# stevenabreu7/SparseRNNs

Hardware: AMD Instinct MI355X
Metric: frames/sec at w8a16 S5 dim_scale=0.5 (NDNS shape), bit-exact vs CPU fxprun (higher is better)
Workload: dtype int32

## Files before the change

sparsernns_amd/csrc/mfma_fused_body.inc:

```
    CGateArgs a = a_k;
    {
        const int64_t g = blockIdx.y;
        gshift(a.u, g * go.ws); gshift(a.skip, g * go.ws); gshift(a.xs, g * go.ws); gshift(a.z, g * go.ws);
        gshift(a.skip_e.dyn, g * go.ws); gshift(a.dynw, g * go.ws); gshift(a.run_if, g * go.ws); gshift(a.status, g * go.status);
        if constexpr (GBN || UREC) { gshift(a.bn.dyn, g * go.ws); gshift(a.bn.xe.dyn, g * go.ws); }
    }
    static_assert(!GBN || (PK16 && !TRACE && !WIDE), "the BatchNorm rides on the packed-epilogue kernel only");
    static_assert(!UREC || (PK16 && !TRACE && !WIDE && !GBN), "u is rebuilt in the row tiles' staging: COAL only");
    constexpr int P = 32 * KS, H = shape_channels(NT), HP = 32 * NT, FT = FTP, NW = (FT / 32) * NT, NTHR = 64 * NW;
    constexpr bool RAGGED = H != HP;
    constexpr int KPS = 2 * P + 16, KPX = HP + 16;
    constexpr int NU = 1, SUBSTEP = 0;
    constexpr int ITEMS = (FT / 4) * P, ROUNDS = (ITEMS + NTHR - 1) / NTHR;
    extern __shared__ __attribute__((aligned(16))) int8_t smem[];
    int32_t *csr = reinterpret_cast<int32_t *>(smem), *csi = csr + HP, *Dl = csi + HP, *cs2 = Dl + HP, *be = cs2 + HP, *lutp = be + HP;
    int32_t *sigt = lutp + 8;
    const int16_t *sigd = reinterpret_cast<const int16_t *>(sigt);
    constexpr int NPL = WIDE ? 4 : 2;
    int8_t *Sbase = reinterpret_cast<int8_t *>(sigt) + (DIRECT ? sigdir_lds_bytes(a.sigdir_bits) : 4 * SIGTAB_WORDS);
    int8_t *Sl = Sbase, *Sh = Sbase + (NPL - 1) * FT * KPS, *Xh = Sbase + NPL * FT * KPS, *Xl = Xh + FT * KPX;
    float *red = reinterpret_cast<float *>(Xl + FT * KPX);
    int32_t *bntab = reinterpret_cast<int32_t *>(red + 48);
    constexpr bool COAL = PK16 && !TRACE && !WIDE && !GBN;
    constexpr int TROW = 2 * HP + 8, VPF = H / 8, NVC = (FT * VPF + NTHR - 1) / NTHR;
    constexpr bool NVC_FULL = FT * VPF % NTHR == 0;
    static_assert(!COAL || NVC_FULL || RAGGED, "tile vectors per thread");
    static_assert(!UREC || NTHR % VPF == 0, "a thread's channel group must be the same for every vector");
    static_assert(!FOLD || (UREC && !RAGGED), "the aligned sum is formed in the UREC staging");
    int8_t *Ut = reinterpret_cast<int8_t *>(red + 48), *St = Ut + FT * TROW;
    const int l = threadIdx.x & 63, r = l & 31, h = l >> 5, wave = threadIdx.x >> 6;
    const int ct = wave % NT, sub0 = wave / NT;
    const StepRange sr{a.t_lo, a.t_len};
    const int64_t tiles = (a.N / a.L) * ((sr.t_len + FT - 1) / FT);
    if (WIDE && a.run_if && *a.run_if == 0) return;

    v4i wre[KS], wim[KS], wo2[NT];
    {
        const size_t row = (size_t)(32 * ct + r);
#pragma unroll
        for (int ks = 0; ks < KS; ++ks) {
            wre[ks] = *reinterpret_cast<const v4i *>(a.w_re.wt + row * a.w_re.Kp + 32 * ks + 16 * h);
            wim[ks] = *reinterpret_cast<const v4i *>(a.w_im.wt + row * a.w_im.Kp + 32 * ks + 16 * h);
        }
#pragma unroll
        for (int ks = 0; ks < NT; ++ks) wo2[ks] = *reinterpret_cast<const v4i *>(a.w_o2.wt + row * a.w_o2.Kp + 32 * ks + 16 * h);
    }
    for (int i = threadIdx.x; i < HP; i += NTHR) {
        csr[i] = a.w_re.cs128[i]; csi[i] = a.w_im.cs128[i]; Dl[i] = a.D[i]; cs2[i] = a.w_o2.cs128[i];
        if (!PK16) be[i] = a.bias_eff[i];
    }
    if (PK16)
        for (int i = threadIdx.x; i < HP / 2; i += NTHR)
            be[i] = (int32_t)(((uint32_t)a.bias_eff[2 * i] & 0xffffu) | ((uint32_t)a.bias_eff[2 * i + 1] << 16));
    if (threadIdx.x < 8) lutp[threadIdx.x] = a_k.lut[threadIdx.x] | (a_k.lut[threadIdx.x < 7 ? threadIdx.x + 1 : 7] << 16);
    if (DIRECT) {
        for (int i = threadIdx.x; i < (1 << a.sigdir_bits) / 2; i += NTHR)
            sigt[i] = reinterpret_cast<const int32_t *>(a.sigdir)[i];
    } else {
        for (int i = threadIdx.x; i < (14 << a.sig_x); i += NTHR) sigt[i] = a.sigtab[i];
    }
    Bn16 bn{};
    if constexpr (GBN) bn = bn16_setup(a.bn, *a.bn.dyn, bntab, H);
    std::conditional_t<UREC, Bn16Row, int> brow{};
    if constexpr (UREC) brow = bn16_row_setup(a.bn, *a.bn.dyn, 8 * (int)(threadIdx.x % VPF));
    [[maybe_unused]] v4i *brow_lds = reinterpret_cast<v4i *>(St + FT * TROW);
    if constexpr (FOLD) {
        if (threadIdx.x < VPF) {
            brow_lds[2 * threadIdx.x] = v4i{(int)brow.m[0], (int)brow.m[1], (int)brow.m[2], (int)brow.m[3]};
            brow_lds[2 * threadIdx.x + 1] = v4i{(int)brow.iv[0], (int)brow.iv[1], (int)brow.iv[2], (int)brow.iv[3]};
        }
    }
    const int dsh = a.out_exp - a.sig_x, dbias = 1 << (a.sigdir_bits - 1);
    const int skip_e = a.skip_e.get();
    const float kz = ldexpf(1.f, skip_e - a.res_exp);
    const v4i *usum_lds = reinterpret_cast<const v4i *>(red + 8);
    if constexpr (FOLD) {
        if (threadIdx.x == 0) {
            const SumU16 us = sum_u16_setup_exps(a.res_exp, skip_e);
            *reinterpret_cast<v4i *>(red + 8) = v4i{(int)us.mz, (int)us.mz2, (int)us.ms, (int)us.ms2};
            const LayerDyn *sd = skip_dyn_of(a_k);
            gshift(sd, (int64_t)blockIdx.y * go.ws);
            const ResolveU16 rz = resolve_u16_setup(sd ? sd->res.post : 0);
            *reinterpret_cast<v4i *>(red + 12) = v4i{(int)rz.shr, (int)rz.m1, (int)rz.m2, sd ? 1 : 0};
        }
    }
    auto resolve_skip = [&](v4i &sv) {
        const v4i rw = *reinterpret_cast<const v4i *>(red + 12);
        if (__builtin_amdgcn_readfirstlane(rw[3])) {
            const ResolveU16 rz{(uint32_t)rw[0], (uint32_t)rw[1], (uint32_t)rw[2], RES_GENERIC};
#pragma unroll
            for (int q = 0; q < 4; ++q) sv[q] = (int)resolve_u16_pair<RES_GENERIC>(rz, (uint32_t)sv[q]);
        }
    };
    const int sx = a.sig_x, S = 1 << sx;
    const int cv_l = a.conv && a.inp_exp > a.y_exp ? a.inp_exp - a.y_exp : 0, cv_r = a.conv && a.y_exp > a.inp_exp ? a.y_exp - a.inp_exp : 0;
    const int cv_b1 = a.conv && a.inp_exp != a.y_exp ? a.y_bits : 32, cv_b2 = a.conv && a.y_bits > a.inp_bits ? a.inp_bits : 32;
    const int cv_b = cv_b1 < cv_b2 ? cv_b1 : cv_b2;
    const int lq_l = a.l_exp > a.y_exp ? a.l_exp - a.y_exp : 0, lq_r = a.y_exp > a.l_exp ? a.y_exp - a.l_exp : 0;
    uint32_t xrange = 0;
    v2i16 pmax = {0, 0}, pmin = {0, 0};
    float mx[3] = {0.f, 0.f, 0.f};
    const int ch0 = 32 * ct + 4 * h;
    v2i uq[NU][4], sq[NU][4];
    v4i urow[COAL && !UREC ? NVC : 1], srow[COAL ? NVC : 1];
    auto load_tile = [&](v4i(&dst)[COAL ? NVC : 1], const int16_t *src, const TileWalk<FT> &tw) {
        const int64_t b = tw.b;
        const int t = tw.t(sr), nv = tw.nvalid(sr);
        const char *base = reinterpret_cast<const char *>(src + (b * a.L + t) * H);
#pragma unroll
        for (int i = 0; i < NVC; ++i) {
            const int v = threadIdx.x + NTHR * i;
            if (!NVC_FULL && v >= FT * VPF) break;
            int f = v / VPF;
            f = f < nv ? f : nv - 1;
            dst[i] = *reinterpret_cast<const v4i *>(base + 2u * (unsigned)(f * H + 8 * (v % VPF)));
        }
    };
    auto load_rows = [&](v2i(&dst)[NU][4], const int16_t *src, const TileWalk<FT> &tw) {
        const int64_t b = tw.b;
        const int t = tw.t(sr), nv = tw.nvalid(sr);
        const char *base = reinterpret_cast<const char *>(src + (b * a.L + t) * H);
#pragma unroll
        for (int u = 0; u < NU; ++u) {
            int fo = 32 * (sub0 + u * SUBSTEP) + r;
            fo = fo < nv ? fo : nv - 1;
            const unsigned fb = 2u * (unsigned)(fo * H + ch0);
#pragma unroll
            for (int g = 0; g < 4; ++g) {
                if (RAGGED && ch0 + 8 * g >= H) dst[u][g] = v2i{0, 0};
                else dst[u][g] = *reinterpret_cast<const v2i *>(base + fb + 16 * g);
            }
        }
    };
    if constexpr (COAL && RAGGED) {
        for (int i = threadIdx.x; i < 2 * FT; i += NTHR) {
            int8_t *t = Ut + i * TROW + 2 * H;
#pragma unroll
            for (int j = 0; j < (HP - H) / 4; ++j) *reinterpret_cast<v2i *>(t + 8 * j) = v2i{0, 0};
        }
    }
    TileWalk<FT> walk((int64_t)blockIdx.x, sr, gridDim.x);
    if ((int64_t)blockIdx.x < tiles) {
        if constexpr (COAL) {
            if constexpr (!UREC) load_tile(urow, a.u, walk);
            load_tile(srow, a.skip, walk);
        } else {
            if constexpr (!GBN) load_rows(uq, a.u, walk);
            load_rows(sq, a.skip, walk);
        }
    }
    __syncthreads();
    char *zb_prev = nullptr;
    int nvalid_prev = 0;
    auto fold_z = [&](v2i &z0, v2i &z1, const int8_t *cs_) {
        const v2i s0 = *reinterpret_cast<const v2i *>(cs_), s1 = *reinterpret_cast<const v2i *>(cs_ + 8);
        const v4i uw = *usum_lds;
        const SumU16 usum{(uint32_t)uw[0], (uint32_t)uw[1], (uint32_t)uw[2], (uint32_t)uw[3]};
#pragma unroll
        for (int q = 0; q < 2; ++q) {
            z0[q] = (int)sum_u16_pair(usum, (uint32_t)z0[q], (uint32_t)s0[q]);
            z1[q] = (int)sum_u16_pair(usum, (uint32_t)z1[q], (uint32_t)s1[q]);
        }
    };
    uint32_t elo[4] = {0xffffffffu, 0xffffffffu, 0xffffffffu, 0xffffffffu}, ehi[4] = {0u, 0u, 0u, 0u};
    auto ext_u = [&](const v2i &z0, const v2i &z1) {
#pragma unroll
        for (int q = 0; q < 2; ++q) {
            elo[q] = pk_min_u(elo[q], (uint32_t)z0[q]); ehi[q] = pk_max_u(ehi[q], (uint32_t)z0[q]);
            elo[2 + q] = pk_min_u(elo[2 + q], (uint32_t)z1[q]); ehi[2 + q] = pk_max_u(ehi[2 + q], (uint32_t)z1[q]);
        }
    };
    auto tiles_in_out = [&](bool incoming) {
#pragma unroll
        for (int i = 0; i < NVC; ++i) {
            const int v = threadIdx.x + NTHR * i, f = v / VPF, og = v % VPF;
            if (!NVC_FULL && v >= FT * VPF) break;
            int8_t *cu = Ut + f * TROW + 16 * og, *cs_ = St + f * TROW + 16 * og;
            if (zb_prev) {
                v2i z0 = *reinterpret_cast<const v2i *>(cu), z1 = *reinterpret_cast<const v2i *>(cu + 8);
                if constexpr (FOLD) fold_z(z0, z1, cs_);
                if (f < nvalid_prev) {
                    *reinterpret_cast<v4i *>(zb_prev + 2u * (unsigned)(f * H + 8 * og)) = v4i{z0[0], z0[1], z1[0], z1[1]};
                    if constexpr (FOLD) ext_u(z0, z1);
                }
            }
            if (incoming) {
                const v4i &uv = urow[UREC ? 0 : i];
                *reinterpret_cast<v2i *>(cu) = v2i{uv[0], uv[1]};
                *reinterpret_cast<v2i *>(cu + 8) = v2i{uv[2], uv[3]};
                *reinterpret_cast<v2i *>(cs_) = v2i{srow[i][0], srow[i][1]};
                *reinterpret_cast<v2i *>(cs_ + 8) = v2i{srow[i][2], srow[i][3]};
            }
        }
    };
    auto tiles_in_urec = [&](auto arm_c) {
        constexpr int ARM = decltype(arm_c)::value;
        auto br = brow;
        if constexpr (FOLD) {
            const v4i bm = brow_lds[2 * (threadIdx.x % VPF)], bi = brow_lds[2 * (threadIdx.x % VPF) + 1];
#pragma unroll
            for (int k = 0; k < 4; ++k) { br.m[k] = (uint32_t)bm[k]; br.iv[k] = (uint32_t)bi[k]; }
        }
#pragma unroll
        for (int i = 0; i < NVC; ++i) {
            const int v = threadIdx.x + NTHR * i, f = v / VPF, og = v % VPF;
            if (!NVC_FULL && v >= FT * VPF) break;
            int8_t *cu = Ut + f * TROW + 16 * og, *cs_ = St + f * TROW + 16 * og;
            if (zb_prev) {
                v2i z0 = *reinterpret_cast<const v2i *>(cu), z1 = *reinterpret_cast<const v2i *>(cu + 8);
                if constexpr (FOLD) fold_z(z0, z1, cs_);
                if (f < nvalid_prev) {
                    *reinterpret_cast<v4i *>(zb_prev + 2u * (unsigned)(f * H + 8 * og)) = v4i{z0[0], z0[1], z1[0], z1[1]};
                    if constexpr (FOLD) ext_u(z0, z1);
                }
            }
            if constexpr (FOLD) resolve_skip(srow[i]);
            const v4i uv = bn16_row8<ARM>(br, srow[i]);
            *reinterpret_cast<v2i *>(cu) = v2i{uv[0], uv[1]};
            *reinterpret_cast<v2i *>(cu + 8) = v2i{uv[2], uv[3]};
            *reinterpret_cast<v2i *>(cs_) = v2i{srow[i][0], srow[i][1]};
            *reinterpret_cast<v2i *>(cs_ + 8) = v2i{srow[i][2], srow[i][3]};
        }
    };

    prologue_loads_done();
    for (int64_t tile = blockIdx.x; tile < tiles; tile += gridDim.x, walk.advance()) {
        const int64_t b0 = walk.b;
        const int t0 = walk.t(sr), nvalid = walk.nvalid(sr);
        const TileWalk<FT> walk_next = walk.next();
        const int64_t n0 = b0 * a.L + t0;
        char *zb = reinterpret_cast<char *>(a.z + n0 * H);
        const int64_t tile_next = tile + gridDim.x;
        if constexpr (UREC) {
            if (brow.arm == ROW_PACKED) tiles_in_urec(std::integral_constant<int, ROW_PACKED>{});
            else if (brow.arm == ROW_SHIFTED) tiles_in_urec(std::integral_constant<int, ROW_SHIFTED>{});
            else tiles_in_urec(std::integral_constant<int, ROW_GENERIC>{});
        } else if constexpr (COAL) tiles_in_out(true);
#pragma unroll
        for (int i = 0; i < ROUNDS; ++i) {
            const int q = threadIdx.x + NTHR * i;
            if (ROUNDS * NTHR == ITEMS || q < ITEMS) {
                const int grp = q / P, p = q % P;
                int o = 4 * grp;
                if (o >= nvalid) o = (nvalid - 1) & ~3;
                const int nlive = nvalid - o;
                int32_t w[4];
                if (WIDE) {
                    const int32_t *src = a.xs + native_word(b0, t0 + o, p, 0, a.TB, P);
                    const v4i cre = *reinterpret_cast<const v4i *>(src), cim = *reinterpret_cast<const v4i *>(src + 4);
                    int32_t xr[4] = {cre[0], cre[1], cre[2], cre[3]}, xi[4] = {cim[0], cim[1], cim[2], cim[3]};
#pragma unroll
                    for (int j = 0; j < 4; ++j) crelu(xr[j], xi[j]);
                    quad_transpose(xr, l);
                    quad_transpose(xi, l);
                    const int row = (4 * grp + (l & 3)) * KPS + (p & ~3);
#pragma unroll
                    for (int c = 0; c < 2; ++c) {
                        const int32_t(&v)[4] = c ? xi : xr;
                        const unsigned t01 = perm((unsigned)v[1], (unsigned)v[0], 0x05010400u), u01 = perm((unsigned)v[1], (unsigned)v[0], 0x07030602u);
                        const unsigned t23 = perm((unsigned)v[3], (unsigned)v[2], 0x05010400u), u23 = perm((unsigned)v[3], (unsigned)v[2], 0x07030602u);
                        int8_t *dst = Sbase + row + c * P;
                        *reinterpret_cast<int32_t *>(dst) = (int32_t)(perm(t23, t01, 0x05040100u) ^ 0x80808080u);
                        *reinterpret_cast<int32_t *>(dst + FT * KPS) = (int32_t)(perm(t23, t01, 0x07060302u) ^ 0x80808080u);
                        *reinterpret_cast<int32_t *>(dst + 2 * FT * KPS) = (int32_t)(perm(u23, u01, 0x05040100u) ^ 0x80808080u);
                        *reinterpret_cast<int32_t *>(dst + 3 * FT * KPS) = (int32_t)perm(u23, u01, 0x07060302u);
                    }
                    continue;
                }
                if (S16) {
                    if (PAIR) {
                        const char *xb = reinterpret_cast<const char *>(reinterpret_cast<const int16_t *>(a.xs) + (pair_word(b0, t0 >> 3, 0, a.TB >> 1, P) << 1));
                        const unsigned xo = 2u * (unsigned)((((((p >> 5) * (a.TB >> 1) + (o >> 3)) << 5) + (p & 31)) << 4) + (o & 4));
                        v2i qa = {0, 0}, qb = {0, 0};
                        if (a.live_slots <= 0 || p < a.live_slots) {
                            qa = *reinterpret_cast<const v2i *>(xb + xo); qb = *reinterpret_cast<const v2i *>(xb + xo + 16);
                        }
                        w[0] = (int32_t)perm((unsigned)qa[0], (unsigned)qb[0], 0x05040100u);
                        w[1] = (int32_t)perm((unsigned)qb[1], (unsigned)qa[1], 0x05040100u);
                        w[2] = (int32_t)perm((unsigned)qa[0], (unsigned)qb[0], 0x07060302u);
                        w[3] = (int32_t)perm((unsigned)qb[1], (unsigned)qa[1], 0x07060302u);
                    } else {
                    v4i q4 = {0, 0, 0, 0};
                    if (a.live_slots <= 0 || p < a.live_slots)
                        q4 = *reinterpret_cast<const v4i *>(reinterpret_cast<const int16_t *>(a.xs) + native_word(b0, t0 + o, p, 0, a.TB, P));
                    w[0] = (int32_t)perm((unsigned)q4[2], (unsigned)q4[0], 0x05040100u);
                    w[1] = (int32_t)perm((unsigned)q4[2], (unsigned)q4[0], 0x07060302u);
                    w[2] = (int32_t)perm((unsigned)q4[3], (unsigned)q4[1], 0x05040100u);
                    w[3] = (int32_t)perm((unsigned)q4[3], (unsigned)q4[1], 0x07060302u);
                    }
                    if (nlive < 4) {
#pragma unroll
                        for (int j = 1; j < 4; ++j) w[j] = j < nlive ? w[j] : 0;
                    }
#pragma unroll
                    for (int j = 0; j < 4; ++j) {
                        pmax = __builtin_elementwise_max(pmax, __builtin_bit_cast(v2i16, w[j]));
                        pmin = __builtin_elementwise_min(pmin, __builtin_bit_cast(v2i16, w[j]));
                        const bool keep = ((int32_t)((uint32_t)w[j] << 16) + (w[j] >> 16)) > 0;
                        w[j] = keep ? w[j] : 0;
                    }
                } else {
                const int32_t *src = a.xs + native_word(b0, t0 + o, p, 0, a.TB, P);
                const v4i cre = *reinterpret_cast<const v4i *>(src), cim = *reinterpret_cast<const v4i *>(src + 4);
#pragma unroll
                for (int j = 0; j < 4; ++j) {
                    const int32_t xr = j < nlive ? cre[j] : 0, xi = j < nlive ? cim[j] : 0;
                    const uint32_t ur = (uint32_t)(xr + a.xmax), ui = (uint32_t)(xi + a.xmax);
                    xrange = xrange > ur ? xrange : ur;
                    xrange = xrange > ui ? xrange : ui;
                    const bool keep = (xr > 0) | ((xr == 0) & (xi > 0));
                    w[j] = keep ? (int32_t)perm((unsigned)xi, (unsigned)xr, 0x05040100u) : 0;
                }
                }
                quad_transpose(w, l);
                const unsigned t01 = perm((unsigned)w[1], (unsigned)w[0], 0x05010400u), u01 = perm((unsigned)w[1], (unsigned)w[0], 0x07030602u);
                const unsigned t23 = perm((unsigned)w[3], (unsigned)w[2], 0x05010400u), u23 = perm((unsigned)w[3], (unsigned)w[2], 0x07030602u);
                const int row = (4 * grp + (l & 3)) * KPS + (p & ~3);
                *reinterpret_cast<int32_t *>(Sl + row) = (int32_t)(perm(t23, t01, 0x05040100u) ^ 0x80808080u);
                *reinterpret_cast<int32_t *>(Sh + row) = (int32_t)perm(t23, t01, 0x07060302u);
                *reinterpret_cast<int32_t *>(Sl + row + P) = (int32_t)(perm(u23, u01, 0x05040100u) ^ 0x80808080u);
                *reinterpret_cast<int32_t *>(Sh + row + P) = (int32_t)perm(u23, u01, 0x07060302u);
            }
        }
        if constexpr (COAL) {
            if (tile_next < tiles) {
                if constexpr (!UREC) load_tile(urow, a.u, walk_next);
                load_tile(srow, a.skip, walk_next);
            }
        }
        lds_barrier();
        int32_t x1v[NU][16];
        uint32_t x1p[NU][8];
#pragma unroll
        for (int u = 0; u < NU; ++u) {
            const int sub = sub0 + u * SUBSTEP;
            const int64_t n = n0 + 32 * sub + r;
            const int8_t *row0 = Sbase + (32 * sub + r) * KPS + 16 * h;
            v16i are, aim;
            mfma_nplanes<KS, NPL>(are, wre, row0, FT * KPS, csr + ch0);
            mfma_nplanes<KS, NPL>(aim, wim, row0 + P, FT * KPS, csi + ch0);
#pragma unroll
            for (int g = 0; g < 4; ++g) {
                const v4i Dv = *reinterpret_cast<const v4i *>(Dl + ch0 + 8 * g);
                const int off = (32 * sub + r) * KPX + ch0 + 8 * g;
                if constexpr (PK16) {
                    int32_t ubn[4];
                    if constexpr (GBN) {
                        int32_t hin[4], tbn[4];
                        unpack4_i16(sq[u][g], hin);
                        bn16_x4(bn, hin, ch0 + 8 * g, tbn, ubn);
                    }
#pragma unroll
                    for (int q = 0; q < 2; ++q) {
                        const uint32_t crp = pk_cvt(asr(are[4 * g + 2 * q], a.rs_re), asr(are[4 * g + 2 * q + 1], a.rs_re));
                        const uint32_t cip = pk_cvt(asr(aim[4 * g + 2 * q], a.rs_im), asr(aim[4 * g + 2 * q + 1], a.rs_im));
                        uint32_t dup;
                        if constexpr (GBN) {
                            dup = pk_cvt(asr(__mul24(Dv[2 * q], ubn[2 * q]), a.rs_d), asr(__mul24(Dv[2 * q + 1], ubn[2 * q + 1]), a.rs_d));
                        } else {
                            uint32_t upk;
                            if constexpr (COAL) upk = (uint32_t)(*reinterpret_cast<const v2i *>(Ut + (32 * sub + r) * TROW + 2 * (ch0 + 8 * g)))[q];
                            else upk = (uint32_t)uq[u][g][q];
                            dup = pk_cvt(asr(mul24_h<0>(Dv[2 * q], upk), a.rs_d), asr(mul24_h<1>(Dv[2 * q + 1], upk), a.rs_d));
                        }
                        const uint32_t yp = pk_mad_sat(pk_sub_sat(crp, cip), 0x00020002u, dup);
                        x1p[u][2 * g + q] = pk_max(yp, 0u);
                    }
                    const uint32_t p01 = x1p[u][2 * g], p23 = x1p[u][2 * g + 1];
                    *reinterpret_cast<int32_t *>(Xl + off) = (int32_t)(perm(p23, p01, 0x06040200u) ^ 0x80808080u);
                    *reinterpret_cast<int32_t *>(Xh + off) = (int32_t)perm(p23, p01, 0x07050301u);
                } else {
                int32_t uv[4], xv[4];
                unpack4_i16(uq[u][g], uv);
#pragma unroll
                for (int e = 0; e < 4; ++e) {
                    const int32_t cr = sat(asr(are[4 * g + e], a.rs_re), a.y_bits);
                    const int32_t ci = sat(asr(aim[4 * g + e], a.rs_im), a.y_bits);
                    const int32_t cx = sat(cr - ci, a.y_bits);
                    const int32_t du = sat(asr(__mul24(Dv[e], uv[e]), a.rs_d), a.y_bits);
                    const int32_t y = sat(2 * cx + du, a.y_bits);
                    if (TRACE) {
                        if (a.tr_ys && 32 * sub + r < nvalid && (!RAGGED || ch0 + 8 * g < H)) a.tr_ys[n * H + ch0 + 8 * g + e] = y;
                    }
                    const int32_t x1 = y < 0 ? 0 : y;
                    x1v[u][4 * g + e] = x1;
                    xv[e] = x1;
                }
                if (a.conv) {
#pragma unroll
                    for (int e = 0; e < 4; ++e) xv[e] = sat(asr(wshl(xv[e], cv_l), cv_r), cv_b);
                }
                const unsigned p01 = perm((unsigned)xv[1], (unsigned)xv[0], 0x05010400u), p23 = perm((unsigned)xv[3], (unsigned)xv[2], 0x05010400u);
                *reinterpret_cast<int32_t *>(Xl + off) = (int32_t)(perm(p23, p01, 0x05040100u) ^ 0x80808080u);
                *reinterpret_cast<int32_t *>(Xh + off) = (int32_t)perm(p23, p01, 0x07060302u);
                }
            }
        }
        if constexpr (!GBN) {
            if (!COAL && tile_next < tiles) load_rows(uq, a.u, walk_next);
        }
        lds_barrier();
#pragma unroll
        for (int u = 0; u < NU; ++u) {
            const int sub = sub0 + u * SUBSTEP;
            const int64_t n = n0 + 32 * sub + r;
            v16i acc;
            mfma_planes<NT>(acc, wo2, Xh + (32 * sub + r) * KPX + 16 * h, Xl + (32 * sub + r) * KPX + 16 * h, cs2 + ch0);
            auto b2_pk16 = [&]() {
                const uint32_t lm = 0x10001u * (uint32_t)(1 << lq_l), lr = 0x10001u * (uint32_t)lq_r;
#pragma unroll
                for (int g = 0; g < 4; ++g) {
                    const int ch = ch0 + 8 * g;
                    const v2i bp = *reinterpret_cast<const v2i *>(be + (ch >> 1));
                    v2i zo;
#pragma unroll
                    for (int q = 0; q < 2; ++q) {
                        uint32_t gp = pk_cvt(asr(acc[4 * g + 2 * q], a.rs_o2), asr(acc[4 * g + 2 * q + 1], a.rs_o2));
                        gp = pk_add_sat(gp, (uint32_t)bp[q]);
                        const int32_t r0 = sigd[ashr_h<0>(dsh, gp) + dbias], r1 = sigd[ashr_h<1>(dsh, gp) + dbias];
                        uint32_t lp = x1p[u][2 * g + q];
                        lp = pk_ashr_u(pk_mul_sat_u(lp, lm), lr);
                        const uint32_t zp = pk_cvt(asr(mul24_h<0>(r0, lp), a.rs_gate), asr(mul24_h<1>(r1, lp), a.rs_gate));
                        zo[q] = (int)zp;
                        uint32_t sp;
                        if constexpr (COAL) sp = (uint32_t)(*reinterpret_cast<const v2i *>(St + (32 * sub + r) * TROW + 2 * ch))[q];
                        else sp = (uint32_t)sq[u][g][q];
                        mx[0] = fmaxf(mx[0], fabsf(__fmaf_rn(cvtf_h<0>(zp), kz, cvtf_h<0>(sp))));
                        mx[0] = fmaxf(mx[0], fabsf(__fmaf_rn(cvtf_h<1>(zp), kz, cvtf_h<1>(sp))));
                    }
                    if constexpr (COAL) *reinterpret_cast<v2i *>(Ut + (32 * sub + r) * TROW + 2 * ch) = zo;
                    else if (!RAGGED || ch < H) *reinterpret_cast<v2i *>(zb + 2u * (unsigned)((32 * sub + r) * H + ch)) = zo;
                }
            };
            if constexpr (PK16) {
                if (32 * sub + r < nvalid) b2_pk16();
            }
            if (!PK16 && 32 * sub + r < nvalid) {
#pragma unroll
                for (int g = 0; g < 4; ++g) {
                    const int ch = ch0 + 8 * g;
                    const v4i bv = *reinterpret_cast<const v4i *>(be + ch);
                    int32_t sv[4], o[4];
                    unpack4_i16(sq[u][g], sv);
#pragma unroll
                    for (int e = 0; e < 4; ++e) {
                        int32_t gq = sat(asr(acc[4 * g + e], a.rs_o2), a.out_bits);
                        gq = sat(gq + bv[e], a.out_bits);
                        int32_t s = 0, rq;
                        if (DIRECT) {
                            rq = sigd[(gq >> dsh) + dbias];
                        } else {
                        const int32_t xx = chexp(gq, a.out_bits, a.out_exp, sx);
                        const int32_t ax = xx < 0 ? -xx : xx;
                        int32_t ind = ax >> sx;
                        ind = ind > 6 ? 6 : ind;
                        const int32_t mu = ax & (S - 1);
                        if (TRACE) {
                            const uint32_t pr = (uint32_t)lutp[ind];
                            const int32_t half = (__mul24(S - mu, (int32_t)(pr & 0xffffu)) >> sx) + (__mul24(mu, (int32_t)(pr >> 16)) >> sx);
                            s = (1 << (a.sig_y - 1)) + (xx > 0 ? half : -half);
                            rq = chcfg(s, a.out_bits, a.sig_y, a.r_bits, a.r_exp);
                        } else {
                            rq = sigt[((ind << sx) | mu) + (xx > 0 ? 7 * S : 0)];
                        }
                        }
                        const int32_t lq = chcfg(x1v[u][4 * g + e], a.y_bits, a.y_exp, a.l_bits, a.l_exp);
                        const int32_t z = sat(asr(__mul24(lq, rq), a.rs_gate), a.res_bits);
                        if (TRACE && (!RAGGED || ch < H)) {
                            if (a.tr_out2) a.tr_out2[n * H + ch + e] = gq;
                            if (a.tr_sig) a.tr_sig[n * H + ch + e] = s;
                            if (a.tr_z) a.tr_z[n * H + ch + e] = z;
                        }
                        o[e] = z;
                        const float cz = (float)z, cs = (float)sv[e];
                        mx[0] = fmaxf(mx[0], fabsf(__fmaf_rn(cz, kz, cs)));
                    }
                    if (!RAGGED || ch < H) *reinterpret_cast<v2i *>(zb + 2u * (unsigned)((32 * sub + r) * H + ch)) = pack4_i16(o[0], o[1], o[2], o[3]);
                }
            }
        }
        if constexpr (COAL) {
            zb_prev = zb; nvalid_prev = nvalid;
            lds_barrier();
        } else {
            if (tile_next < tiles) load_rows(sq, a.skip, walk_next);
        }
    }
    if constexpr (COAL) tiles_in_out(false);
    [[maybe_unused]] float *ext_next = nullptr;
    [[maybe_unused]] uint32_t *ext_lds = reinterpret_cast<uint32_t *>(Ut);
    if constexpr (FOLD) {
        static_assert(2 * NTHR * 16 <= 2 * FT * TROW, "the parked extremes fit the two tiles");
        ext_next = ext_next_of(a_k);
        if (ext_next) {
            __syncthreads();
#pragma unroll
            for (int q = 0; q < 2; ++q) {
                *reinterpret_cast<v2i *>(ext_lds + 4 * threadIdx.x + 2 * q) = v2i{(int)elo[2 * q], (int)elo[2 * q + 1]};
                *reinterpret_cast<v2i *>(ext_lds + 4 * (NTHR + threadIdx.x) + 2 * q) = v2i{(int)ehi[2 * q], (int)ehi[2 * q + 1]};
            }
        }
    }
    if (S16) {
        const int hi = pmax[0] > pmax[1] ? pmax[0] : pmax[1], lo = pmin[0] < pmin[1] ? pmin[0] : pmin[1];
        if (hi > a.xmax || lo < -a.xmax) xrange = 0xffffffffu;
    }
    if (__any(xrange > 2u * (uint32_t)a.xmax) && l == 0) {
        atomicExch(&a.dynw->redo, 1);
        atomicOr(a.status, a.bad_bits);
    }
    mx[0] = ldexpf(mx[0], -skip_e);
    mx[1] = ldexpf(mx[1], -a.res_exp);
    mx[2] = ldexpf(mx[2], -skip_e);
#pragma unroll
    for (int i = 0; i < 3; ++i) {
        float x = mx[i];
#pragma unroll
        for (int o = 32; o > 0; o >>= 1) x = fmaxf(x, __shfl_xor(x, o, 64));
        if (l == 0) red[i * 16 + wave] = x;
    }
    __syncthreads();
    if (threadIdx.x < 3) {
        float x = red[threadIdx.x * 16];
        for (int w = 1; w < NW; ++w) x = fmaxf(x, red[threadIdx.x * 16 + w]);
        atomicMax(a.dynw->mx + a.mx_slot + threadIdx.x, __float_as_uint(x));
    }
    if constexpr (FOLD) {
        if (ext_next && (int64_t)blockIdx.x < tiles) {
            gshift_nn(ext_next, (int64_t)blockIdx.y * go.ws);
            for (int item = threadIdx.x; item < 2 * H; item += NTHR) {
                const bool is_max = item >= H;
                const int c = is_max ? item - H : item;
                const uint16_t *src = reinterpret_cast<const uint16_t *>(ext_lds + (is_max ? 4 * NTHR : 0)) + 8 * (c >> 3) + (c & 7);
                int32_t v = is_max ? 0 : 65535;
#pragma unroll 4
                for (int k = 0; k < NTHR / VPF; ++k) {
                    const int32_t t = src[8 * VPF * k];
                    v = is_max ? max(v, t) : min(v, t);
                }
                atomicMax(reinterpret_cast<uint32_t *>(ext_next) + (int)(blockIdx.x % EXT_REPS) * 2 * H + item,
                          __float_as_uint(is_max ? EXT_BIAS + (float)v : EXT_BIAS - (float)v));
            }
        }
    }
```

sparsernns_amd/csrc/scan_quad.hpp:

```cpp
#pragma once
#include "fxp_prims.hpp"

namespace s5 {

using u32x4 = __attribute__((__vector_size__(4 * sizeof(unsigned int)))) unsigned int;
using i32x4 = __attribute__((ext_vector_type(4))) int;

struct GroupOff {
    int64_t x, y, ws, status, state_in, state_out;
};
using gchar = __attribute__((address_space(1))) char;
template <class P>
__device__ __forceinline__ P as_global(P p)
{
    return (P)(char *)(gchar *)(char *)p;
}
template <class P>
__device__ __forceinline__ void gshift(P &p, int64_t bytes)
{
    p = p ? (P)(char *)((gchar *)(char *)p + bytes) : (P) nullptr;
}
template <class P>
__device__ __forceinline__ void gshift_nn(P &p, int64_t bytes)
{
    p = (P)(char *)((gchar *)(char *)p + bytes);
}

__device__ __forceinline__ void prologue_loads_done() { __builtin_amdgcn_s_waitcnt(0x0F70); }

using v4i_ = __attribute__((ext_vector_type(4))) int;
__device__ __forceinline__ v4i_ gload16_hidden(const char *base, unsigned off)
{
    v4i_ r;
    asm volatile("global_load_dwordx4 %0, %1, %2" : "=&v"(r) : "v"(off), "s"(base) : "memory");
    return r;
}
using v2i_ = __attribute__((ext_vector_type(2))) int;
__device__ __forceinline__ v2i_ gload8_hidden(const char *base, unsigned off)
{
    v2i_ r;
    asm volatile("global_load_dwordx2 %0, %1, %2" : "=&v"(r) : "v"(off), "s"(base) : "memory");
    return r;
}
template <class V> __device__ __forceinline__ V gload_hidden(const char *base, unsigned off)
{
    if constexpr (sizeof(V) == 16) return gload16_hidden(base, off);
    else return gload8_hidden(base, off);
}
template <int NEWER, class T, int N>
__device__ __forceinline__ void vm_wait(T (&regs)[N])
{
    static_assert(NEWER >= 0 && NEWER < 64, "vmcnt is a 6-bit counter");
    asm volatile("s_waitcnt vmcnt(%0)" : : "n"(NEWER) : "memory");
#pragma unroll
    for (int i = 0; i < N; ++i) asm volatile("" : "+v"(regs[i]));
}

__device__ __forceinline__ int64_t native_word(int64_t b, int t, int p, int c, int TB, int P)
{
    return ((((b * TB + (t >> 2)) * P + p) * 2 + c) << 2) + (t & 3);
}

struct CarryCheck {
    int32_t xmax, bad_bits;
    int32_t *redo;
    int32_t *status;
};
__device__ __forceinline__ void carry_check(CarryCheck c, const GroupOff &go, int32_t x0)
{
    if (c.xmax <= 0) return;
    if (__any(x0 > c.xmax || x0 < -c.xmax) && (threadIdx.x & 63) == 0) {
        const int64_t g = blockIdx.y;
        gshift_nn(c.redo, g * go.ws); gshift_nn(c.status, g * go.status);
        atomicExch(c.redo, 1);
        atomicOr(c.status, c.bad_bits);
    }
}

struct ScanQuadArgs {
    const int32_t *bq;
    int32_t *xs;
    const int32_t *a_re, *a_im;
    int32_t B, TB, P;
    int32_t ea_re, ea_im;
    int32_t tb0, ntb;
    const int32_t *run_if;
    const int32_t *x0_re, *x0_im;
    int32_t live_slots;
    CarryCheck cc;
};

__device__ __forceinline__ int32_t quad_x0(const ScanQuadArgs &a, int b, int p, int r)
{
    if (!a.x0_re) return 0;
    return (r == 0 || r == 3) ? a.x0_re[(size_t)b * a.P + p] : a.x0_im[(size_t)b * a.P + p];
}

#define S5_SCAN_STEP(PRE, PERM, XIN, XOUT, C, K, BQ)                                                           \
    asm volatile(PRE "v_mad_i32_i24 %0, %2, %3, %4\n\t"                                                          \
                 "v_add_u32_sdwa %0, sext(%0), %5 dst_sel:DWORD dst_unused:UNUSED_PAD src0_sel:WORD_1 "        \
                 "src1_sel:DWORD\n\t"                                                                          \
                 "s_nop 1\n\t"                                                                                 \
                 "v_add_u32_dpp %1, %0, %0 quad_perm:" PERM " row_mask:0xf bank_mask:0xf\n\t"                  \
                 : "=&v"(tmp), "=v"(XOUT)                                                                      \
                 : "v"(C), "v"(XIN), "v"(K), "v"(BQ))

template <int DEPTH>
__global__ __launch_bounds__(256) void k_scan_quad(ScanQuadArgs a)
{
    const int lane = threadIdx.x & 63, wave_in_block = threadIdx.x >> 6;
    const int wave = __builtin_amdgcn_readfirstlane(blockIdx.x * 4 + wave_in_block);
    const int groups = a.P >> 4;
    const int b = wave / groups, p0 = (wave % groups) << 4;
    if (b >= a.B) return;
    const int s = lane >> 2, r = lane & 3;
    const int p = p0 + s;
    const int32_t Ar = a.a_re[p], Ai = a.a_im[p];
    const int sre = 16 - a.ea_re, sim = 16 - a.ea_im;
    const int32_t kre = (1 << 16) - (1 << sre);
    int32_t cA, cB, kA = 0, kB = 0;
    if (r == 0) { cA = cB = Ar << sre; }
    else if (r == 1) { cA = cB = Ar << sim; }
    else if (r == 2) { cA = -(Ai << sre); kA = kre; cB = Ai << sim; }
    else { cA = Ai << sim; cB = -(Ai << sre); kB = kre; }

    const size_t wave_off = (((size_t)b * a.TB) * a.P + p0) * 8;
    const unsigned blk_stride = (unsigned)a.P * 32u;
    const unsigned extent = (unsigned)a.TB * blk_stride;
    auto rin = __builtin_amdgcn_make_buffer_rsrc(const_cast<int32_t *>(a.bq) + wave_off, 0, extent, 0x00020000);
    auto rout = __builtin_amdgcn_make_buffer_rsrc(a.xs + wave_off, 0, extent, 0x00020000);
    const unsigned voff = r < 2 ? (unsigned)(s * 32 + r * 16) : 0xFFFFFF00u;

    u32x4 ring[DEPTH];
    unsigned soff_ld = 0, soff_st = 0;
#pragma unroll
    for (int i = 0; i < DEPTH; ++i) {
        ring[i] = __builtin_amdgcn_raw_buffer_load_b128(rin, voff, soff_ld, 0);
        soff_ld += blk_stride;
    }
    int32_t x = 0, tmp;
    for (int tb0 = 0; tb0 < a.TB; tb0 += DEPTH) {
#pragma unroll
        for (int i = 0; i < DEPTH; ++i) {
            const u32x4 cur = ring[i];
            int32_t x1, x2, x3, x4;
            S5_SCAN_STEP("s_nop 1\n\t", "[2,3,0,1]", x, x1, cA, kA, cur[0]);
            S5_SCAN_STEP("", "[3,2,1,0]", x1, x2, cB, kB, cur[1]);
            S5_SCAN_STEP("", "[2,3,0,1]", x2, x3, cA, kA, cur[2]);
            S5_SCAN_STEP("", "[3,2,1,0]", x3, x4, cB, kB, cur[3]);
            x = x4;
            ring[i] = __builtin_amdgcn_raw_buffer_load_b128(rin, voff, soff_ld < extent ? soff_ld : extent - blk_stride, 0);
            soff_ld += blk_stride;
            u32x4 o;
            o[0] = (unsigned)x1; o[1] = (unsigned)x2; o[2] = (unsigned)x3; o[3] = (unsigned)x4;
            __builtin_amdgcn_raw_buffer_store_b128(o, rout, voff, soff_st, 0);
            soff_st += blk_stride;
        }
    }
}

#include "scan_quad_asm.inc"

__device__ __forceinline__ void scan_quad_group(ScanQuadArgs &a, const GroupOff &go)
{
    const int64_t g = blockIdx.y;
    gshift(a.bq, g * go.ws); gshift(a.xs, g * go.ws); gshift(a.run_if, g * go.ws);
    gshift(a.x0_re, g * go.state_in); gshift(a.x0_im, g * go.state_in);
}

__global__ __launch_bounds__(64) void k_scan_quad_asm(ScanQuadArgs a, GroupOff go)
{
    scan_quad_group(a, go);
    const int lane = threadIdx.x & 63;
    const int wave = __builtin_amdgcn_readfirstlane((int)blockIdx.x);
    const int groups = a.P >> 4;
    const int b = wave / groups, p0 = (wave % groups) << 4;
    if (b >= a.B) return;
    const int s = lane >> 2, r = lane & 3;
    const int p = p0 + s;
    const int32_t Ar = a.a_re[p], Ai = a.a_im[p];
    const int sre = 16 - a.ea_re, sim = 16 - a.ea_im;
    const int32_t kre = (1 << 16) - (1 << sre);
    int32_t cA, cB, kA = 0, kB = 0;
    if (r == 0) { cA = cB = Ar << sre; }
    else if (r == 1) { cA = cB = Ar << sim; }
    else if (r == 2) { cA = -(Ai << sre); kA = kre; cB = Ai << sim; }
    else { cA = Ai << sim; cB = -(Ai << sre); kB = kre; }
    const int tb0 = a.tb0, ntb = a.ntb > 0 ? a.ntb : a.TB - a.tb0;
    int32_t x0 = quad_x0(a, b, p, r);
    carry_check(a.cc, go, x0);
    if (tb0 > 0) x0 = a.xs[native_word(b, 4 * tb0 - 1, p, (r == 0 || r == 3) ? 0 : 1, a.TB, a.P)];
    const size_t wave_off = (((size_t)b * a.TB + tb0) * a.P + p0) * 8;
    const unsigned blk_stride = (unsigned)a.P * 32u;
    const unsigned extent = (unsigned)(a.TB - tb0) * blk_stride;
    const unsigned long long bin = (unsigned long long)(a.bq + wave_off), bout = (unsigned long long)(a.xs + wave_off);
    u32x4 rin, rout;
    rin[0] = (unsigned)bin; rin[1] = (unsigned)(bin >> 32) & 0xffffu; rin[2] = extent; rin[3] = 0x00020000u;
    rout[0] = (unsigned)bout; rout[1] = (unsigned)(bout >> 32) & 0xffffu; rout[2] = extent; rout[3] = 0x00020000u;
    const unsigned voff = r < 2 ? (unsigned)(s * 32 + r * 16) : 0xFFFFFF00u;
    unsigned sld = 0, sst = 0, cnt = (unsigned)ntb / S5_SCAN_ASM_DEPTH;
    asm volatile(S5_SCAN_ASM_BODY
                 : [sld] "+s"(sld), [sst] "+s"(sst), [cnt] "+s"(cnt)
                 : [ca] "v"(cA), [cb] "v"(cB), [ka] "v"(kA), [kb] "v"(kB), [voff] "v"(voff), [x0] "v"(x0), [rin] "s"(rin),
                   [rout] "s"(rout), [stride] "s"(blk_stride)
                 : S5_SCAN_ASM_CLOBBERS);
}

__global__ __launch_bounds__(64) void k_scan_quad_asm16(ScanQuadArgs a, GroupOff go)
{
    scan_quad_group(a, go);
    const int lane = threadIdx.x & 63;
    const int wave = __builtin_amdgcn_readfirstlane((int)blockIdx.x);
    const int groups = a.P >> 4;
    const int b = wave / groups, p0 = (wave % groups) << 4;
    if (b >= a.B) return;
    const int s = lane >> 2, r = lane & 3;
    const int p = p0 + s;
    const int32_t Ar = a.a_re[p], Ai = a.a_im[p];
    const int sre = 16 - a.ea_re, sim = 16 - a.ea_im;
    const int32_t kre = (1 << 16) - (1 << sre);
    int32_t cA, cB, kA = 0, kB = 0;
    if (r == 0) { cA = cB = Ar << sre; }
    else if (r == 1) { cA = cB = Ar << sim; }
    else if (r == 2) { cA = -(Ai << sre); kA = kre; cB = Ai << sim; }
    else { cA = Ai << sim; cB = -(Ai << sre); kB = kre; }
    const int32_t x0 = quad_x0(a, b, p, r);
    carry_check(a.cc, go, x0);
    const size_t wave_off = (((size_t)b * a.TB) * a.P + p0) * 8;
    const unsigned blk_stride = (unsigned)a.P * 16u;
    const unsigned extent = (unsigned)a.TB * blk_stride;
    const unsigned long long bin = (unsigned long long)(reinterpret_cast<const int16_t *>(a.bq) + wave_off),
                             bout = (unsigned long long)(reinterpret_cast<int16_t *>(a.xs) + wave_off);
    u32x4 rin, rout;
    rin[0] = (unsigned)bin; rin[1] = (unsigned)(bin >> 32) & 0xffffu; rin[2] = extent; rin[3] = 0x00020000u;
    rout[0] = (unsigned)bout; rout[1] = (unsigned)(bout >> 32) & 0xffffu; rout[2] = extent; rout[3] = 0x00020000u;
    const unsigned voff = r < 2 && (a.live_slots <= 0 || p < a.live_slots) ? (unsigned)(s * 16 + r * 8) : 0xFFFFFF00u;
    unsigned sld = 0, sst = 0, cnt = (unsigned)a.TB / S5_SCAN_ASM_DEPTH;
    asm volatile(S5_SCAN16_ASM_BODY
                 : [sld] "+s"(sld), [sst] "+s"(sst), [cnt] "+s"(cnt)
                 : [ca] "v"(cA), [cb] "v"(cB), [ka] "v"(kA), [kb] "v"(kB), [voff] "v"(voff), [x0] "v"(x0), [rin] "s"(rin),
                   [rout] "s"(rout), [stride] "s"(blk_stride)
                 : S5_SCAN16_ASM_CLOBBERS);
}

__global__ __launch_bounds__(64) void k_scan_quad32_asm(ScanQuadArgs a, GroupOff go)
{
    scan_quad_group(a, go);
    if (a.run_if && *a.run_if == 0) return;
    const int lane = threadIdx.x & 63;
    const int wave = __builtin_amdgcn_readfirstlane((int)blockIdx.x);
    const int groups = a.P >> 4;
    const int b = wave / groups, p0 = (wave % groups) << 4;
    if (b >= a.B) return;
    const int s = lane >> 2, r = lane & 3;
    const int p = p0 + s;
    const int32_t Ar = a.a_re[p], Ai = a.a_im[p];
    int32_t cA, cB, sA, sB, mA = 0, mB = 0;
    if (r == 0) { cA = cB = Ar; sA = sB = a.ea_re; }
    else if (r == 1) { cA = cB = Ar; sA = sB = a.ea_im; }
    else if (r == 2) { cA = cB = Ai; sA = a.ea_re; mA = -1; sB = a.ea_im; }
    else { cA = cB = Ai; sA = a.ea_im; sB = a.ea_re; mB = -1; }
    const int32_t oA = mA & 1, oB = mB & 1, x0 = quad_x0(a, b, p, r);
    const size_t wave_off = (((size_t)b * a.TB) * a.P + p0) * 8;
    const unsigned blk_stride = (unsigned)a.P * 32u;
    const unsigned extent = (unsigned)a.TB * blk_stride;
    const unsigned long long bin = (unsigned long long)(a.bq + wave_off), bout = (unsigned long long)(a.xs + wave_off);
    u32x4 rin, rout;
    rin[0] = (unsigned)bin; rin[1] = (unsigned)(bin >> 32) & 0xffffu; rin[2] = extent; rin[3] = 0x00020000u;
    rout[0] = (unsigned)bout; rout[1] = (unsigned)(bout >> 32) & 0xffffu; rout[2] = extent; rout[3] = 0x00020000u;
    const unsigned voff = r < 2 ? (unsigned)(s * 32 + r * 16) : 0xFFFFFF00u;
    unsigned sld = 0, sst = 0, cnt = (unsigned)a.TB / S5_SCAN_ASM_DEPTH;
    asm volatile(S5_SCAN32W_ASM_BODY
                 : [sld] "+s"(sld), [sst] "+s"(sst), [cnt] "+s"(cnt)
                 : [ca] "v"(cA), [cb] "v"(cB), [sa] "v"(sA), [sb] "v"(sB), [ma] "v"(mA), [mb] "v"(mB), [oa] "v"(oA),
                   [ob] "v"(oB), [voff] "v"(voff), [x0] "v"(x0), [rin] "s"(rin), [rout] "s"(rout), [stride] "s"(blk_stride)
                 : S5_SCAN32W_ASM_CLOBBERS);
}

__device__ __forceinline__ int64_t pair_word(int64_t b, int tb, int p, int TB, int P)
{
    return ((((b * (P >> 5) + (p >> 5)) * TB + tb) << 5) + (p & 31)) << 3;
}

__global__ void k_state_out(const void *xs, int mode, const int32_t *redo, int B, int L, int P, int TB, int32_t *out_re,
                            int32_t *out_im, GroupOff go)
{
    {
        const int64_t g = blockIdx.y;
        gshift(xs, g * go.ws); gshift(redo, g * go.ws); gshift(out_re, g * go.state_out); gshift(out_im, g * go.state_out);
    }
    const int i = blockIdx.x * blockDim.x + threadIdx.x;
    if (i >= B * P) return;
    const int b = i / P, p = i % P, t = L - 1;
    if (redo && *redo) mode = 0;
    int32_t re, im;
    if (mode == 0) {
        const int32_t *x = reinterpret_cast<const int32_t *>(xs);
        re = x[native_word(b, t, p, 0, TB, P)];
        im = x[native_word(b, t, p, 1, TB, P)];
    } else if (mode == 1) {
        const int16_t *x = reinterpret_cast<const int16_t *>(xs);
        re = x[native_word(b, t, p, 0, TB, P)];
        im = x[native_word(b, t, p, 1, TB, P)];
    } else {
        const int16_t *x = reinterpret_cast<const int16_t *>(xs) + (pair_word(b, t >> 3, p, TB >> 1, P) << 1);
        const int j = t & 7, jj = j & 3;
        const int hw = (2 * (j >> 2) + (jj & 1)) * 2 + (jj >> 1);
        const int16_t va = x[hw], vb = x[8 + hw];
        re = (j & 1) ? va : vb;
        im = (j & 1) ? vb : va;
    }
    out_re[i] = re;
    out_im[i] = im;
}

struct ScanPairArgs {
    const int32_t *k;
    int16_t *xs;
    const int32_t *a_re, *a_im;
    int32_t B, TB, P;
    int32_t ea_re, ea_im;
    const int32_t *x0_re, *x0_im;
    CarryCheck cc;
};

__global__ __launch_bounds__(64) void k_scan_pair_asm(ScanPairArgs a, GroupOff go)
{
    {
        const int64_t g = blockIdx.y;
        gshift(a.k, g * go.ws); gshift(a.xs, g * go.ws); gshift(a.x0_re, g * go.state_in); gshift(a.x0_im, g * go.state_in);
    }
    const int lane = threadIdx.x & 63;
    const int wave = __builtin_amdgcn_readfirstlane((int)blockIdx.x);
    if (wave >= a.B * (a.P >> 5)) return;
    const int p = ((wave % (a.P >> 5)) << 5) + (lane >> 1);
    const int32_t Ar = a.a_re[p], Ai = a.a_im[p];
    const int sre = 16 - a.ea_re, sim = 16 - a.ea_im;
    const bool laneB = lane & 1;
    const int32_t c_im_own = Ai << sim, c_im_part = Ar << sim, c_re_own = -(Ai << sre), c_re_part = Ar << sre;
    const int32_t coe = laneB ? c_re_own : c_im_own, cpe = laneB ? c_re_part : c_im_part;
    const int32_t coo = laneB ? c_im_own : c_re_own, cpo = laneB ? c_im_part : c_re_part;
    const unsigned long long pin = (unsigned long long)(a.k + (size_t)wave * a.TB * 256),
                             pout = (unsigned long long)(a.xs + (size_t)wave * a.TB * 256);
    const unsigned vin = lane * 16 + 4096, vout = vin;
    const size_t sp = (size_t)(wave / (a.P >> 5)) * a.P + p;
    const int32_t x0 = a.x0_re ? (laneB ? a.x0_im[sp] : a.x0_re[sp]) : 0;
    carry_check(a.cc, go, x0);
    unsigned cnt = (unsigned)a.TB / S5_SCANP_ASM_DEPTH;
    asm volatile(S5_SCANP_ASM_BODY
                 : [cnt] "+s"(cnt)
                 : [coe] "v"(coe), [cpe] "v"(cpe), [coo] "v"(coo), [cpo] "v"(cpo), [vin] "v"(vin), [vout] "v"(vout),
                   [x0] "v"(x0), [pin] "s"(pin), [pout] "s"(pout)
                 : S5_SCANP_ASM_CLOBBERS);
}

__device__ __forceinline__ int64_t pair16_half(int64_t b, int tb, int p, int lane_sel, int TB, int P)
// ... 180 lines not shown
```

Measured before the change: 781.8 million.

## Issue x-state global loads before u-row rebuild and precompute item map

For the UREC/S16/KS=1/FT=32 configuration, the per-thread work item (group, slot) is packed into a register once, and padding slots beyond live_slots are pre-filled in LDS. Each tile's x-state global loads are then issued before the u-row staging work, with a custom vmcnt wait that drains fully when the previous tile was partial. The intent is to hide global load latency behind the row rebuild and to skip dead slots. In exchange it adds register pressure and inline-asm waitcnt logic whose correctness depends on the exact count of outstanding loads.

New measurement: 812.2 million (median of 6 runs). 1.04x the previous value.

```diff
diff --git a/sparsernns_amd/csrc/mfma_fused_body.inc b/sparsernns_amd/csrc/mfma_fused_body.inc
--- a/sparsernns_amd/csrc/mfma_fused_body.inc
+++ b/sparsernns_amd/csrc/mfma_fused_body.inc
@@ -139,6 +139,25 @@
             for (int j = 0; j < (HP - H) / 4; ++j) *reinterpret_cast<v2i *>(t + 8 * j) = v2i{0, 0};
         }
     }
+    constexpr bool EARLY = UREC && S16 && KS == 1 && FT == 32;
+    [[maybe_unused]] uint32_t items = 0;
+    static_assert(!EARLY || (ROUNDS <= 2 && FT / 4 <= 8), "a half-word per round: three bits of group, the slot above them");
+    [[maybe_unused]] auto item_of = [&](int i) { return (int)((items >> (16 * i)) & 0xffffu); };
+    if constexpr (EARLY) {
+        const int PL = a.live_slots > 0 ? (a.live_slots + 3) & ~3 : P;
+#pragma unroll
+        for (int i = 0; i < ROUNDS; ++i) {
+            const int q = threadIdx.x + NTHR * i, grp = q / PL;
+            items |= (uint32_t)(q < (FT / 4) * PL ? grp | ((q - grp * PL) << 3) : 0xffff) << (16 * i);
+        }
+        for (int i = threadIdx.x; i < FT * ((P - PL) >> 2); i += NTHR) {
+            const int f = i / ((P - PL) >> 2), c = PL + 4 * (i % ((P - PL) >> 2));
+            *reinterpret_cast<int32_t *>(Sl + f * KPS + c) = (int32_t)0x80808080u;
+            *reinterpret_cast<int32_t *>(Sh + f * KPS + c) = 0;
+            *reinterpret_cast<int32_t *>(Sl + f * KPS + P + c) = (int32_t)0x80808080u;
+            *reinterpret_cast<int32_t *>(Sh + f * KPS + P + c) = 0;
+        }
+    }
     TileWalk<FT> walk((int64_t)blockIdx.x, sr, gridDim.x);
     if ((int64_t)blockIdx.x < tiles) {
         if constexpr (COAL) {
@@ -231,13 +250,86 @@
         const int64_t n0 = b0 * a.L + t0;
         char *zb = reinterpret_cast<char *>(a.z + n0 * H);
         const int64_t tile_next = tile + gridDim.x;
+        constexpr int XW = PAIR ? 2 : 1;
+        [[maybe_unused]] std::conditional_t<PAIR, v2i, v4i> xq[EARLY ? XW * ROUNDS : 1] = {};
+        [[maybe_unused]] const bool full_prev = zb_prev && nvalid_prev == FT;
+        auto item_offset = [&](int i, int &o) {
+            const int it = item_of(i), grp = it & 7;
+            int p = it >> 3;
+            p = it != 0xffff && (a.live_slots <= 0 || p < a.live_slots) ? p : 0;
+            o = 4 * grp;
+            if (o >= nvalid) o = (nvalid - 1) & ~3;
+            return PAIR ? 2u * (unsigned)(((((o >> 3) << 5) + p) << 4) + (o & 4)) : 16u * (unsigned)((o >> 2) * P + p);
+        };
+        if constexpr (EARLY) {
+            prologue_loads_done();
+            const char *xb = reinterpret_cast<const char *>(reinterpret_cast<const int16_t *>(a.xs) +
+                                                            (PAIR ? pair_word(b0, t0 >> 3, 0, a.TB >> 1, P) << 1 : native_word(b0, t0, 0, 0, a.TB, P)));
+#pragma unroll
+            for (int i = 0; i < ROUNDS; ++i) {
+                if (i > 0 && __builtin_amdgcn_readfirstlane(item_of(i)) == 0xffff) break;
+                int o;
+                const unsigned xo = item_offset(i, o);
+                if constexpr (PAIR) { xq[2 * i] = gload8_hidden(xb, xo); xq[2 * i + 1] = gload8_hidden(xb, xo + 16); }
+                else xq[i] = gload16_hidden(xb, xo);
+            }
+        }
         if constexpr (UREC) {
             if (brow.arm == ROW_PACKED) tiles_in_urec(std::integral_constant<int, ROW_PACKED>{});
             else if (brow.arm == ROW_SHIFTED) tiles_in_urec(std::integral_constant<int, ROW_SHIFTED>{});
             else tiles_in_urec(std::integral_constant<int, ROW_GENERIC>{});
+            if constexpr (EARLY) {
+                vm_wait_or_drain<NVC>(full_prev, xq);
+            }
         } else if constexpr (COAL) tiles_in_out(true);
-#pragma unroll
-        for (int i = 0; i < ROUNDS; ++i) {
+        if constexpr (EARLY) {
+#pragma unroll
+            for (int i = 0; i < ROUNDS; ++i) {
+                if (i > 0 && __builtin_amdgcn_readfirstlane(item_of(i)) == 0xffff) break;
+                if (item_of(i) != 0xffff) {
+                    const int grp = item_of(i) & 7, p = item_of(i) >> 3;
+                    int o;
+                    item_offset(i, o);
+                    const int nlive = nvalid - o;
+                    const bool held = a.live_slots <= 0 || p < a.live_slots;
+                    int32_t w[4];
+                    if constexpr (PAIR) {
+                        const v2i qa = held ? xq[2 * i] : v2i{0, 0}, qb = held ? xq[2 * i + 1] : v2i{0, 0};
+                        w[0] = (int32_t)perm((unsigned)qa[0], (unsigned)qb[0], 0x05040100u);
+                        w[1] = (int32_t)perm((unsigned)qb[1], (unsigned)qa[1], 0x05040100u);
+                        w[2] = (int32_t)perm((unsigned)qa[0], (unsigned)qb[0], 0x07060302u);
+                        w[3] = (int32_t)perm((unsigned)qb[1], (unsigned)qa[1], 0x07060302u);
+                    } else {
+                        const v4i q4 = held ? xq[i] : v4i{0, 0, 0, 0};
+                        w[0] = (int32_t)perm((unsigned)q4[2], (unsigned)q4[0], 0x05040100u);
+                        w[1] = (int32_t)perm((unsigned)q4[2], (unsigned)q4[0], 0x07060302u);
+                        w[2] = (int32_t)perm((unsigned)q4[3], (unsigned)q4[1], 0x05040100u);
+                        w[3] = (int32_t)perm((unsigned)q4[3], (unsigned)q4[1], 0x07060302u);
+                    }
+                    if (nlive < 4) {
+#pragma unroll
+                        for (int j = 1; j < 4; ++j) w[j] = j < nlive ? w[j] : 0;
+                    }
+#pragma unroll
+                    for (int j = 0; j < 4; ++j) {
+                        pmax = __builtin_elementwise_max(pmax, __builtin_bit_cast(v2i16, w[j]));
+                        pmin = __builtin_elementwise_min(pmin, __builtin_bit_cast(v2i16, w[j]));
+                        const bool keep = ((int32_t)((uint32_t)w[j] << 16) + (w[j] >> 16)) > 0;
+                        w[j] = keep ? w[j] : 0;
+                    }
+                    quad_transpose(w, l);
+                    const unsigned t01 = perm((unsigned)w[1], (unsigned)w[0], 0x05010400u), u01 = perm((unsigned)w[1], (unsigned)w[0], 0x07030602u);
+                    const unsigned t23 = perm((unsigned)w[3], (unsigned)w[2], 0x05010400u), u23 = perm((unsigned)w[3], (unsigned)w[2], 0x07030602u);
+                    const int row = (4 * grp + (l & 3)) * KPS + (p & ~3);
+                    *reinterpret_cast<int32_t *>(Sl + row) = (int32_t)(perm(t23, t01, 0x05040100u) ^ 0x80808080u);
+                    *reinterpret_cast<int32_t *>(Sh + row) = (int32_t)perm(t23, t01, 0x07060302u);
+                    *reinterpret_cast<int32_t *>(Sl + row + P) = (int32_t)(perm(u23, u01, 0x05040100u) ^ 0x80808080u);
+                    *reinterpret_cast<int32_t *>(Sh + row + P) = (int32_t)perm(u23, u01, 0x07060302u);
+                }
+            }
+        }
+#pragma unroll
+        for (int i = 0; i < (EARLY ? 0 : ROUNDS); ++i) {
             const int q = threadIdx.x + NTHR * i;
             if (ROUNDS * NTHR == ITEMS || q < ITEMS) {
                 const int grp = q / P, p = q % P;
@@ -512,18 +604,21 @@
     mx[0] = ldexpf(mx[0], -skip_e);
     mx[1] = ldexpf(mx[1], -a.res_exp);
     mx[2] = ldexpf(mx[2], -skip_e);
+    unsigned tx = threadIdx.x;
+    if constexpr (EARLY) asm volatile("" : "+v"(tx));
+    const int wave_r = EARLY ? (int)(tx >> 6) : wave;
 #pragma unroll
     for (int i = 0; i < 3; ++i) {
         float x = mx[i];
 #pragma unroll
         for (int o = 32; o > 0; o >>= 1) x = fmaxf(x, __shfl_xor(x, o, 64));
-        if (l == 0) red[i * 16 + wave] = x;
+        if (l == 0) red[i * 16 + wave_r] = x;
     }
     __syncthreads();
-    if (threadIdx.x < 3) {
-        float x = red[threadIdx.x * 16];
-        for (int w = 1; w < NW; ++w) x = fmaxf(x, red[threadIdx.x * 16 + w]);
-        atomicMax(a.dynw->mx + a.mx_slot + threadIdx.x, __float_as_uint(x));
+    if (tx < 3) {
+        float x = red[tx * 16];
+        for (int w = 1; w < NW; ++w) x = fmaxf(x, red[tx * 16 + w]);
+        atomicMax(a.dynw->mx + a.mx_slot + tx, __float_as_uint(x));
     }
     if constexpr (FOLD) {
         if (ext_next && (int64_t)blockIdx.x < tiles) {
diff --git a/sparsernns_amd/csrc/scan_quad.hpp b/sparsernns_amd/csrc/scan_quad.hpp
--- a/sparsernns_amd/csrc/scan_quad.hpp
+++ b/sparsernns_amd/csrc/scan_quad.hpp
@@ -52,6 +52,18 @@
 {
     static_assert(NEWER >= 0 && NEWER < 64, "vmcnt is a 6-bit counter");
     asm volatile("s_waitcnt vmcnt(%0)" : : "n"(NEWER) : "memory");
+#pragma unroll
+    for (int i = 0; i < N; ++i) asm volatile("" : "+v"(regs[i]));
+}
+
+template <int NEWER, class T, int N>
+__device__ __forceinline__ void vm_wait_or_drain(bool counted, T (&regs)[N])
+{
+    static_assert(NEWER >= 0 && NEWER < 64, "vmcnt is a 6-bit counter");
+    asm volatile("s_cmp_lg_u32 %0, 0\n\ts_cbranch_scc1 1f\n\ts_waitcnt vmcnt(0)\n1:\n\ts_waitcnt vmcnt(%1)"
+                 :
+                 : "s"(__builtin_amdgcn_readfirstlane((int)counted)), "n"(NEWER)
+                 : "memory", "scc");
 #pragma unroll
     for (int i = 0; i < N; ++i) asm volatile("" : "+v"(regs[i]));
 }
```
